# alpa-projects/alpa

Hardware: AMD Instinct MI355X
Metric: model_tflops_aggregate (higher is better)
Workload: dtype bf16; 1 GPU; model=GPT-2.6B, hidden=2560, layers=32, heads=32, vocab=51200, global_batch=32, seq_len=1024, num_micro_batches=1, parallelism=dp1, hip_graph=True

## Files before the change

### alpa_amd/ops/csrc/attention.hip

```cpp
#include "common.h"
#include "launchers.h"

#define ATTN_BLOCK_K 64
#define ATTN_FWD_THREADS 512
#define ATTN_BWD_THREADS 512

struct AttnStrides {
  int64_t qb, qh, qs;
  int64_t kb, kh, ks;
  int64_t vb, vh, vs;
  int64_t ob, oh, os;
};

static AttnStrides attn_strides(const int64_t* s) {
  return {s[0], s[1], s[2], s[3], s[4], s[5],
          s[6], s[7], s[8], s[9], s[10], s[11]};
}

__device__ inline int xcd_swizzle(int flat, int total) {
  constexpr int NXCD = 8;
  if (total % NXCD != 0) return flat;
  return (flat % NXCD) * (total / NXCD) + flat / NXCD;
}

template <int Dp, bool AL = false, bool VL = false>
__global__ __launch_bounds__(ATTN_FWD_THREADS) void attn_fwd_kernel(
    const short* __restrict__ q, const short* __restrict__ k,
    const short* __restrict__ v, short* __restrict__ o,
    float* __restrict__ lse_out, int H, int S, int Skv, int D, float scale,
    int causal, const float* __restrict__ alibi,
    const int* __restrict__ kv_lens, AttnStrides st) {
  constexpr bool DB = Dp <= 128;
  constexpr int NT = ATTN_FWD_THREADS;
  constexpr int KSTEPS_QK = Dp / 32;
  constexpr int NTILES = ATTN_BLOCK_K / 16;
  constexpr int DTILES = Dp / 16;
  constexpr int LP = 4;
  constexpr int NW = NT / 64;
  constexpr int GPR = Dp / 8;
  constexpr int TOTAL_G = ATTN_BLOCK_K * GPR;
  constexpr int G_PER_T = (TOTAL_G + NT - 1) / NT;

  const int flat_ = xcd_swizzle(
      (int)(blockIdx.y * gridDim.x + blockIdx.x),
      (int)(gridDim.x * gridDim.y));
  const int qb_raw = flat_ % (int)gridDim.x;
  const int qb = causal ? ((int)gridDim.x - 1 - qb_raw) : qb_raw;
  const int bh = flat_ / (int)gridDim.x;
  const int batch = bh / H, head = bh % H;
  const int wave = threadIdx.x >> 6;
  const int lane = threadIdx.x & 63;
  const int lo = lane & 15;
  const int hi = lane >> 4;

  const short* qp = q + batch * st.qb + head * st.qh;
  const short* kp = k + batch * st.kb + head * st.kh;
  const short* vp = v + batch * st.vb + head * st.vh;
  short* op = o + batch * st.ob + head * st.oh;
  const int q_row0 = qb * (16 * NW) + wave * 16;

  __shared__ short k_lds[DB ? 2 : 1][ATTN_BLOCK_K][Dp + LP];
  __shared__ short vt_lds[DB ? 2 : 1][Dp][ATTN_BLOCK_K + LP];
  __shared__ short p_lds[NW][16][ATTN_BLOCK_K + LP];

  bf16x8 q_frag[KSTEPS_QK];
  {
    int row = min(q_row0 + lo, S - 1);
#pragma unroll
    for (int ks = 0; ks < KSTEPS_QK; ++ks) {
      int col = ks * 32 + hi * 8;
      bf16x8 z = {0, 0, 0, 0, 0, 0, 0, 0};
      q_frag[ks] = z;
      if (col + 8 <= D)
        q_frag[ks] =
            *reinterpret_cast<const bf16x8*>(qp + (int64_t)row * st.qs + col);
    }
  }

  float m_state = -INFINITY, l_state = 0.f;
  f32x4 o_acc[DTILES];
#pragma unroll
  for (int dt = 0; dt < DTILES; ++dt) o_acc[dt] = f32x4{0.f, 0.f, 0.f, 0.f};

  const int kv_limit =
      causal ? min(Skv, qb * (16 * NW) + 16 * NW) : Skv;
  const int n_tiles = (kv_limit + ATTN_BLOCK_K - 1) / ATTN_BLOCK_K;
  const int my_q = q_row0 + lo;
  const int my_skv = VL ? kv_lens[batch] : Skv;
  const float al_slope = AL ? alibi[bh % H] : 0.f;
  const int al_qoff = my_skv - S;

  bf16x8 kreg[2 * G_PER_T], vreg[2 * G_PER_T];
  auto issue_loads = [&](int tile) {
#pragma unroll
    for (int it = 0; it < G_PER_T; ++it) {
      int t = threadIdx.x + it * NT;
      bf16x8 z = {0, 0, 0, 0, 0, 0, 0, 0};
      kreg[2 * it] = z; kreg[2 * it + 1] = z;
      vreg[2 * it] = z; vreg[2 * it + 1] = z;
      if (t < TOTAL_G / 2) {
        int kvr = (t / GPR) * 2, dg = (t % GPR) * 8;
#pragma unroll
        for (int u = 0; u < 2; ++u) {
          int src = tile * ATTN_BLOCK_K + kvr + u;
          if (src < Skv && dg + 8 <= D) {
            kreg[2 * it + u] = *reinterpret_cast<const bf16x8*>(
                kp + (int64_t)src * st.ks + dg);
            vreg[2 * it + u] = *reinterpret_cast<const bf16x8*>(
                vp + (int64_t)src * st.vs + dg);
          }
        }
      }
    }
  };
  auto write_tile = [&](int buf) {
#pragma unroll
    for (int it = 0; it < G_PER_T; ++it) {
      int t = threadIdx.x + it * NT;
      if (t < TOTAL_G / 2) {
        int kvr = (t / GPR) * 2, dg = (t % GPR) * 8;
        *reinterpret_cast<bf16x8*>(&k_lds[buf][kvr][dg]) = kreg[2 * it];
        *reinterpret_cast<bf16x8*>(&k_lds[buf][kvr + 1][dg]) =
            kreg[2 * it + 1];
#pragma unroll
        for (int j = 0; j < 8; ++j) {
          short2 pr;
          pr.x = vreg[2 * it][j];
          pr.y = vreg[2 * it + 1][j];
          *reinterpret_cast<short2*>(&vt_lds[buf][dg + j][kvr]) = pr;
        }
      }
    }
  };

  auto advance = [&](int ti, int cur) {
    if (ti + 1 >= n_tiles) return;
    if (DB) {
      write_tile(1 - cur);
      __syncthreads();
    } else {
      __syncthreads();
      issue_loads(ti + 1);
      write_tile(0);
      __syncthreads();
    }
  };

  if (n_tiles > 0) {
    issue_loads(0);
    write_tile(0);
    __syncthreads();
  }

  for (int ti = 0; ti < n_tiles; ++ti) {
    const int kvb = ti * ATTN_BLOCK_K;
    const int cur = DB ? (ti & 1) : 0;
    if (DB && ti + 1 < n_tiles) issue_loads(ti + 1);

    if (causal && kvb > q_row0 + 15) {
      advance(ti, cur);
      continue;
    }

__builtin_amdgcn_s_setprio(1);
    f32x4 s_acc[NTILES];
#pragma unroll
    for (int nt = 0; nt < NTILES; ++nt) {
      f32x4 acc = {0.f, 0.f, 0.f, 0.f};
#pragma unroll
      for (int ks = 0; ks < KSTEPS_QK; ++ks) {
        bf16x8 a = *reinterpret_cast<const bf16x8*>(
            &k_lds[cur][nt * 16 + lo][ks * 32 + hi * 8]);
        acc = __builtin_amdgcn_mfma_f32_16x16x32_bf16(a, q_frag[ks], acc, 0,
                                                      0, 0);
      }
      s_acc[nt] = acc;
    }
    __builtin_amdgcn_s_setprio(0);

    float tile_max = -INFINITY;
#pragma unroll
    for (int nt = 0; nt < NTILES; ++nt) {
#pragma unroll
      for (int r = 0; r < 4; ++r) {
        int kv_idx = kvb + nt * 16 + hi * 4 + r;
        float sv = s_acc[nt][r] * scale;
        if (AL)
          sv = fmaf(al_slope, (float)(kv_idx - my_q - al_qoff), sv);
        bool masked = (kv_idx >= my_skv) || (causal && kv_idx > my_q) ||
                      (my_q >= S);
        sv = masked ? -INFINITY : sv;
        s_acc[nt][r] = sv;
        tile_max = fmaxf(tile_max, sv);
      }
    }
    tile_max = fmaxf(tile_max, __shfl_xor(tile_max, 16, 64));
    tile_max = fmaxf(tile_max, __shfl_xor(tile_max, 32, 64));

    constexpr float DEFER_THR = 8.0f;
    if (!__all(tile_max <= m_state + DEFER_THR)) {
      float m_new = fmaxf(m_state, tile_max);
      float alpha = (m_state == -INFINITY) ? 0.f : __expf(m_state - m_new);
      m_state = m_new;
      l_state *= alpha;
#pragma unroll
      for (int dt = 0; dt < DTILES; ++dt) {
        o_acc[dt][0] *= alpha; o_acc[dt][1] *= alpha;
        o_acc[dt][2] *= alpha; o_acc[dt][3] *= alpha;
      }
    }
    float part = 0.f;
#pragma unroll
    for (int nt = 0; nt < NTILES; ++nt) {
      bf16x4 pk;
#pragma unroll
      for (int r = 0; r < 4; ++r) {
        float pval = (s_acc[nt][r] == -INFINITY)
                         ? 0.f
                         : __expf(s_acc[nt][r] - m_state);
        part += pval;
        pk[r] = f2bf(pval);
      }
      *reinterpret_cast<bf16x4*>(&p_lds[wave][lo][nt * 16 + hi * 4]) = pk;
    }
    part += __shfl_xor(part, 16, 64);
    part += __shfl_xor(part, 32, 64);
    l_state += part;

__builtin_amdgcn_s_setprio(1);
#pragma unroll
    for (int ks = 0; ks < ATTN_BLOCK_K / 32; ++ks) {
      bf16x8 b = *reinterpret_cast<const bf16x8*>(
          &p_lds[wave][lo][ks * 32 + hi * 8]);
#pragma unroll
      for (int dt = 0; dt < DTILES; ++dt) {
        bf16x8 a = *reinterpret_cast<const bf16x8*>(
            &vt_lds[cur][dt * 16 + lo][ks * 32 + hi * 8]);
        o_acc[dt] =
            __builtin_amdgcn_mfma_f32_16x16x32_bf16(a, b, o_acc[dt], 0, 0, 0);
      }
    }
    __builtin_amdgcn_s_setprio(0);

    advance(ti, cur);
  }

  {
    int q_idx = q_row0 + lo;
    if (q_idx < S) {
      float inv_l = (l_state > 0.f) ? 1.0f / l_state : 0.f;
#pragma unroll
      for (int dt = 0; dt < DTILES; ++dt) {
#pragma unroll
        for (int r = 0; r < 4; ++r) {
          int col = dt * 16 + hi * 4 + r;
          if (col < D)
            op[(int64_t)q_idx * st.os + col] = f2bf(o_acc[dt][r] * inv_l);
        }
      }
      if (hi == 0 && lse_out != nullptr)
        lse_out[(int64_t)bh * S + q_idx] =
            (l_state > 0.f) ? m_state + __logf(l_state) : -INFINITY;
    }
  }
}

extern "C" {

hipError_t launch_attn_fwd(const void* q, const void* k, const void* v,
                           void* o, float* lse, int64_t B, int64_t H,
                           int64_t S, int64_t Skv, int64_t D, float scale,
                           int causal, const float* alibi,
                           const int* kv_lens, const int64_t* strides,
                           hipStream_t stream) {
  const AttnStrides st = attn_strides(strides);
  dim3 grid((uint32_t)ceil_div(S, 16 * (ATTN_FWD_THREADS / 64)),
            (uint32_t)(B * H));
  dim3 block(ATTN_FWD_THREADS);
#define FWD_LAUNCH(DP, ALB, VLB)                                           \
  attn_fwd_kernel<DP, ALB, VLB><<<grid, block, 0, stream>>>(               \
      (const short*)q, (const short*)k, (const short*)v, (short*)o, lse,   \
      (int)H, (int)S, (int)Skv, (int)D, scale, causal, alibi, kv_lens, st)
#define FWD_DISPATCH(DP)                                                   \
  do {                                                                     \
    if (alibi && kv_lens) FWD_LAUNCH(DP, true, true);                      \
    else if (alibi) FWD_LAUNCH(DP, true, false);                           \
    else if (kv_lens) FWD_LAUNCH(DP, false, true);                         \
    else FWD_LAUNCH(DP, false, false);                                     \
  } while (0)
  if (D <= 64) {
    FWD_DISPATCH(64);
  } else if (D <= 96) {
    FWD_DISPATCH(96);
  } else if (D <= 128) {
    FWD_DISPATCH(128);
  } else if (D <= 256 && !alibi && !kv_lens) {
    FWD_LAUNCH(256, false, false);
  } else {
    return hipErrorInvalidValue;
  }
#undef FWD_DISPATCH
#undef FWD_LAUNCH
  return hipGetLastError();
}

}


struct AttnBwdStrides {
  int64_t qb, qh, qs;
  int64_t kb, kh, ks;
  int64_t vb, vh, vs;
  int64_t dob, doh, dos;
  int64_t dqb, dqh, dqs;
  int64_t dkb, dkh, dks;
  int64_t dvb, dvh, dvs;
};

static AttnBwdStrides attn_bwd_strides(const int64_t* s) {
  return {s[0],  s[1],  s[2],  s[3],  s[4],  s[5],  s[6],
          s[7],  s[8],  s[9],  s[10], s[11], s[12], s[13],
          s[14], s[15], s[16], s[17], s[18], s[19], s[20]};
}

__global__ void attn_bwd_preprocess_kernel(const short* __restrict__ dout,
                                           const short* __restrict__ o,
                                           float* __restrict__ delta,
                                           int64_t rows, int H, int S, int D,
                                           int64_t dob, int64_t doh,
                                           int64_t dos, int64_t ob,
                                           int64_t oh, int64_t os) {
  int64_t row = (int64_t)blockIdx.x * (blockDim.x >> 4) + (threadIdx.x >> 4);
  if (row >= rows) return;
  int lane16 = threadIdx.x & 15;
  int64_t sidx = row % S, h = (row / S) % H, b = row / ((int64_t)S * H);
  const short* dr = dout + b * dob + h * doh + sidx * dos;
  const short* orow = o + b * ob + h * oh + sidx * os;
  float s = 0.f;
  for (int i = lane16 * 8; i + 8 <= D; i += 16 * 8) {
    bf16x8 dv = *reinterpret_cast<const bf16x8*>(dr + i);
    bf16x8 ov = *reinterpret_cast<const bf16x8*>(orow + i);
#pragma unroll
    for (int j = 0; j < 8; ++j) s += bf2f(dv[j]) * bf2f(ov[j]);
  }
  if (lane16 == 0)
    for (int i = (D / 8) * 8; i < D; ++i)
      s += bf2f(dr[i]) * bf2f(orow[i]);
#pragma unroll
  for (int off = 8; off > 0; off >>= 1) s += __shfl_xor(s, off, 64);
  if (lane16 == 0) delta[row] = s;
}

template <int Dp, bool AL = false>
__global__ __launch_bounds__(ATTN_BWD_THREADS) void attn_bwd_dq_kernel(
    const short* __restrict__ q, const short* __restrict__ k,
    const short* __restrict__ v, const short* __restrict__ dout,
    const float* __restrict__ lse, const float* __restrict__ delta,
    short* __restrict__ dq, int H, int S, int Skv, int D, float scale,
    int causal, const float* __restrict__ alibi, AttnBwdStrides st) {
  constexpr int KD = Dp / 32;
  constexpr int NT = 4;
  constexpr int DT = Dp / 16;
  constexpr int LP = 4;
  constexpr int NW = ATTN_BWD_THREADS / 64;
  constexpr int GPR = Dp / 8;
  constexpr int PAIRS = 32 * GPR;

  const int flat_ = xcd_swizzle(
      (int)(blockIdx.y * gridDim.x + blockIdx.x),
      (int)(gridDim.x * gridDim.y));
  const int qb_raw = flat_ % (int)gridDim.x;
  const int qb = causal ? ((int)gridDim.x - 1 - qb_raw) : qb_raw;
  const int bh = flat_ / (int)gridDim.x;
  const int batch = bh / H, head = bh % H;
  const int wave = threadIdx.x >> 6;
  const int lane = threadIdx.x & 63;
  const int lo = lane & 15, hi = lane >> 4;

  const short* qp = q + batch * st.qb + head * st.qh;
  const short* kp = k + batch * st.kb + head * st.kh;
  const short* vp = v + batch * st.vb + head * st.vh;
  const short* dop = dout + batch * st.dob + head * st.doh;
  short* dqp = dq + batch * st.dqb + head * st.dqh;
  const int q_row0 = qb * (16 * NW) + wave * 16;

  __shared__ short k_lds[64][Dp + LP];
  __shared__ short kt_lds[Dp][64 + LP];
  __shared__ short v_lds[64][Dp + LP];
  __shared__ short p_lds[NW][16][64 + LP];

  bf16x8 q_frag[KD], do_frag[KD];
  {
    int row = min(q_row0 + lo, S - 1);
#pragma unroll
    for (int ks = 0; ks < KD; ++ks) {
      int col = ks * 32 + hi * 8;
      bf16x8 z = {0, 0, 0, 0, 0, 0, 0, 0};
      q_frag[ks] = z;
      do_frag[ks] = z;
      if (col + 8 <= D) {
        q_frag[ks] = *reinterpret_cast<const bf16x8*>(
            qp + (int64_t)row * st.qs + col);
        do_frag[ks] = *reinterpret_cast<const bf16x8*>(
            dop + (int64_t)row * st.dos + col);
      }
    }
  }
  float lse_r[4], delta_r[4];
#pragma unroll
  for (int r = 0; r < 4; ++r) {
    int qi = q_row0 + hi * 4 + r;
    lse_r[r] = (qi < S) ? lse[(int64_t)bh * S + qi] : 0.f;
    delta_r[r] = (qi < S) ? delta[(int64_t)bh * S + qi] : 0.f;
  }
  const float al_slope = AL ? alibi[bh % H] : 0.f;

  f32x4 dq_acc[DT];
#pragma unroll
  for (int dt = 0; dt < DT; ++dt) dq_acc[dt] = f32x4{0.f, 0.f, 0.f, 0.f};

  const int kv_limit = causal ? min(Skv, qb * (16 * NW) + 16 * NW) : Skv;
  const int n_tiles = (kv_limit + 63) / 64;

  bf16x8 kreg[2], vreg[2];
  auto issue_loads = [&](int tile) {
    int t = threadIdx.x;
    bf16x8 z = {0, 0, 0, 0, 0, 0, 0, 0};
    kreg[0] = kreg[1] = vreg[0] = vreg[1] = z;
    if (t < PAIRS) {
      int kvr = (t / GPR) * 2, dg = (t % GPR) * 8;
#pragma unroll
      for (int u = 0; u < 2; ++u) {
        int src = tile * 64 + kvr + u;
        if (src < Skv && dg + 8 <= D) {
          kreg[u] = *reinterpret_cast<const bf16x8*>(
              kp + (int64_t)src * st.ks + dg);
          vreg[u] = *reinterpret_cast<const bf16x8*>(
              vp + (int64_t)src * st.vs + dg);
        }
      }
    }
  };
  auto write_tile = [&]() {
    int t = threadIdx.x;
    if (t < PAIRS) {
      int kvr = (t / GPR) * 2, dg = (t % GPR) * 8;
      *reinterpret_cast<bf16x8*>(&k_lds[kvr][dg]) = kreg[0];
      *reinterpret_cast<bf16x8*>(&k_lds[kvr + 1][dg]) = kreg[1];
      *reinterpret_cast<bf16x8*>(&v_lds[kvr][dg]) = vreg[0];
      *reinterpret_cast<bf16x8*>(&v_lds[kvr + 1][dg]) = vreg[1];
#pragma unroll
      for (int j = 0; j < 8; ++j) {
        short2 pr;
        pr.x = kreg[0][j];
        pr.y = kreg[1][j];
        *reinterpret_cast<short2*>(&kt_lds[dg + j][kvr]) = pr;
      }
    }
  };

  if (n_tiles > 0) {
    issue_loads(0);
    write_tile();
    __syncthreads();
  }

  for (int ti = 0; ti < n_tiles; ++ti) {
    const int kvb = ti * 64;
    if (ti + 1 < n_tiles) issue_loads(ti + 1);

    if (causal && kvb > q_row0 + 15) {
      __syncthreads();
      if (ti + 1 < n_tiles) { write_tile(); __syncthreads(); }
      continue;
    }

__builtin_amdgcn_s_setprio(1);
    f32x4 s_acc[NT], dp_acc[NT];
#pragma unroll
    for (int nt = 0; nt < NT; ++nt) {
      f32x4 sa = {0.f, 0.f, 0.f, 0.f}, da = {0.f, 0.f, 0.f, 0.f};
#pragma unroll
      for (int ks = 0; ks < KD; ++ks) {
        bf16x8 bk = *reinterpret_cast<const bf16x8*>(
            &k_lds[nt * 16 + lo][ks * 32 + hi * 8]);
        bf16x8 bv = *reinterpret_cast<const bf16x8*>(
            &v_lds[nt * 16 + lo][ks * 32 + hi * 8]);
        sa = __builtin_amdgcn_mfma_f32_16x16x32_bf16(q_frag[ks], bk, sa, 0,
                                                     0, 0);
        da = __builtin_amdgcn_mfma_f32_16x16x32_bf16(do_frag[ks], bv, da, 0,
                                                     0, 0);
      }
      s_acc[nt] = sa;
      dp_acc[nt] = da;
    }
    __builtin_amdgcn_s_setprio(0);

#pragma unroll
    for (int nt = 0; nt < NT; ++nt) {
      int kv_idx = kvb + nt * 16 + lo;
#pragma unroll
      for (int r = 0; r < 4; ++r) {
        int q_idx = q_row0 + hi * 4 + r;
        bool masked = (kv_idx >= Skv) || (causal && kv_idx > q_idx) ||
                      (q_idx >= S);
        float sraw = s_acc[nt][r] * scale;
        if (AL) sraw = fmaf(al_slope, (float)(kv_idx - q_idx), sraw);
        float pv = masked ? 0.f : __expf(sraw - lse_r[r]);
        float ds = pv * (dp_acc[nt][r] - delta_r[r]) * scale;
        p_lds[wave][hi * 4 + r][nt * 16 + lo] = f2bf(ds);
      }
    }

__builtin_amdgcn_s_setprio(1);
#pragma unroll
    for (int ks = 0; ks < 2; ++ks) {
      bf16x8 a = *reinterpret_cast<const bf16x8*>(
          &p_lds[wave][lo][ks * 32 + hi * 8]);
#pragma unroll
      for (int dt = 0; dt < DT; ++dt) {
        bf16x8 b = *reinterpret_cast<const bf16x8*>(
            &kt_lds[dt * 16 + lo][ks * 32 + hi * 8]);
        dq_acc[dt] = __builtin_amdgcn_mfma_f32_16x16x32_bf16(
            a, b, dq_acc[dt], 0, 0, 0);
      }
    }
    __builtin_amdgcn_s_setprio(0);

    __syncthreads();
    if (ti + 1 < n_tiles) {
      write_tile();
      __syncthreads();
    }
  }

#pragma unroll
  for (int r = 0; r < 4; ++r) {
    int q_idx = q_row0 + hi * 4 + r;
    if (q_idx >= S) continue;
#pragma unroll
    for (int dt = 0; dt < DT; ++dt) {
      int col = dt * 16 + lo;
      if (col < D)
        dqp[(int64_t)q_idx * st.dqs + col] = f2bf(dq_acc[dt][r]);
    }
  }
}

template <int Dp, bool AL = false>
__global__ __launch_bounds__(ATTN_BWD_THREADS) void attn_bwd_dkv_kernel(
    const short* __restrict__ q, const short* __restrict__ k,
    const short* __restrict__ v, const short* __restrict__ dout,
    const float* __restrict__ lse, const float* __restrict__ delta,
    short* __restrict__ dk, short* __restrict__ dv, int H, int S, int Skv,
    int D, float scale, int causal, const float* __restrict__ alibi,
    AttnBwdStrides st) {
  constexpr int KD = Dp / 32;
  constexpr int NT = 4;
  constexpr int DT = Dp / 16;
  constexpr int LP = 4;
  constexpr int NW = ATTN_BWD_THREADS / 64;
  constexpr int GPR = Dp / 8;
  constexpr int PAIRS = 32 * GPR;

  const int flat_ = xcd_swizzle(
      (int)(blockIdx.y * gridDim.x + blockIdx.x),
      (int)(gridDim.x * gridDim.y));
  const int kvb_idx = flat_ % (int)gridDim.x;
  const int bh = flat_ / (int)gridDim.x;
  const int batch = bh / H, head = bh % H;
  const int wave = threadIdx.x >> 6;
  const int lane = threadIdx.x & 63;
  const int lo = lane & 15, hi = lane >> 4;

  const short* qp = q + batch * st.qb + head * st.qh;
  const short* kp = k + batch * st.kb + head * st.kh;
  const short* vp = v + batch * st.vb + head * st.vh;
  const short* dop = dout + batch * st.dob + head * st.doh;
  short* dkp = dk + batch * st.dkb + head * st.dkh;
  short* dvp = dv + batch * st.dvb + head * st.dvh;
  const int kv_row0 = kvb_idx * (16 * NW) + wave * 16;
  const float al_slope = AL ? alibi[bh % H] : 0.f;

  __shared__ short q_lds[64][Dp + LP];
  __shared__ short do_lds[64][Dp + LP];
  __shared__ short qt_lds[Dp][64 + LP];
  __shared__ short dot_lds[Dp][64 + LP];
  __shared__ short p_lds[NW][16][64 + LP];
  __shared__ float lse_lds[64];
  __shared__ float delta_lds[64];

  bf16x8 k_frag[KD], v_frag[KD];
  {
    int row = min(kv_row0 + lo, Skv - 1);
#pragma unroll
    for (int ks = 0; ks < KD; ++ks) {
      int col = ks * 32 + hi * 8;
      bf16x8 z = {0, 0, 0, 0, 0, 0, 0, 0};
      k_frag[ks] = z;
      v_frag[ks] = z;
      if (col + 8 <= D) {
        k_frag[ks] = *reinterpret_cast<const bf16x8*>(
            kp + (int64_t)row * st.ks + col);
        v_frag[ks] = *reinterpret_cast<const bf16x8*>(
            vp + (int64_t)row * st.vs + col);
      }
    }
  }

  f32x4 dk_acc[DT], dv_acc[DT];
#pragma unroll
  for (int dt = 0; dt < DT; ++dt) {
    dk_acc[dt] = f32x4{0.f, 0.f, 0.f, 0.f};
    dv_acc[dt] = f32x4{0.f, 0.f, 0.f, 0.f};
  }

  const int q_start = causal ? kvb_idx * (16 * NW) / 64 * 64 : 0;
  const int n_tiles = (S - q_start + 63) / 64;

  bf16x8 qreg[2], doreg[2];
  float lse_reg, delta_reg;
  auto issue_loads = [&](int tile) {
    int t = threadIdx.x;
    bf16x8 z = {0, 0, 0, 0, 0, 0, 0, 0};
    qreg[0] = qreg[1] = doreg[0] = doreg[1] = z;
    int qb0 = q_start + tile * 64;
    if (t < PAIRS) {
      int qr = (t / GPR) * 2, dg = (t % GPR) * 8;
#pragma unroll
      for (int u = 0; u < 2; ++u) {
        int src = qb0 + qr + u;
        if (src < S && dg + 8 <= D) {
          qreg[u] = *reinterpret_cast<const bf16x8*>(
              qp + (int64_t)src * st.qs + dg);
          doreg[u] = *reinterpret_cast<const bf16x8*>(
              dop + (int64_t)src * st.dos + dg);
        }
      }
    }
    lse_reg = delta_reg = 0.f;
    if (t < 64) {
      int src = qb0 + t;
      if (src < S) {
        lse_reg = lse[(int64_t)bh * S + src];
        delta_reg = delta[(int64_t)bh * S + src];
      }
    }
  };
  auto write_tile = [&]() {
    int t = threadIdx.x;
    if (t < PAIRS) {
      int qr = (t / GPR) * 2, dg = (t % GPR) * 8;
      *reinterpret_cast<bf16x8*>(&q_lds[qr][dg]) = qreg[0];
      *reinterpret_cast<bf16x8*>(&q_lds[qr + 1][dg]) = qreg[1];
      *reinterpret_cast<bf16x8*>(&do_lds[qr][dg]) = doreg[0];
      *reinterpret_cast<bf16x8*>(&do_lds[qr + 1][dg]) = doreg[1];
#pragma unroll
      for (int j = 0; j < 8; ++j) {
        short2 pq, pd;
        pq.x = qreg[0][j];
        pq.y = qreg[1][j];
        pd.x = doreg[0][j];
        pd.y = doreg[1][j];
        *reinterpret_cast<short2*>(&qt_lds[dg + j][qr]) = pq;
        *reinterpret_cast<short2*>(&dot_lds[dg + j][qr]) = pd;
      }
    }
    if (t < 64) {
      lse_lds[t] = lse_reg;
      delta_lds[t] = delta_reg;
    }
  };

  if (n_tiles > 0) {
    issue_loads(0);
    write_tile();
    __syncthreads();
  }

  for (int ti = 0; ti < n_tiles; ++ti) {
    const int qb0 = q_start + ti * 64;
    if (ti + 1 < n_tiles) issue_loads(ti + 1);

    if (causal && qb0 + 63 < kv_row0) {
      __syncthreads();
      if (ti + 1 < n_tiles) { write_tile(); __syncthreads(); }
      continue;
    }

__builtin_amdgcn_s_setprio(1);
    f32x4 st_acc[NT], dpt_acc[NT];
#pragma unroll
    for (int nt = 0; nt < NT; ++nt) {
      f32x4 sa = {0.f, 0.f, 0.f, 0.f}, da = {0.f, 0.f, 0.f, 0.f};
#pragma unroll
      for (int ks = 0; ks < KD; ++ks) {
        bf16x8 bq = *reinterpret_cast<const bf16x8*>(
            &q_lds[nt * 16 + lo][ks * 32 + hi * 8]);
        bf16x8 bd = *reinterpret_cast<const bf16x8*>(
            &do_lds[nt * 16 + lo][ks * 32 + hi * 8]);
        sa = __builtin_amdgcn_mfma_f32_16x16x32_bf16(k_frag[ks], bq, sa, 0,
                                                     0, 0);
        da = __builtin_amdgcn_mfma_f32_16x16x32_bf16(v_frag[ks], bd, da, 0,
                                                     0, 0);
      }
      st_acc[nt] = sa;
      dpt_acc[nt] = da;
    }
    __builtin_amdgcn_s_setprio(0);

    short dst_pk[NT][4];
#pragma unroll
    for (int nt = 0; nt < NT; ++nt) {
      int q_idx = qb0 + nt * 16 + lo;
#pragma unroll
      for (int r = 0; r < 4; ++r) {
        int kv_idx = kv_row0 + hi * 4 + r;
        bool masked = (q_idx >= S) || (kv_idx >= Skv) ||
                      (causal && kv_idx > q_idx);
        float sraw = st_acc[nt][r] * scale;
        if (AL) sraw = fmaf(al_slope, (float)(kv_idx - q_idx), sraw);
        float pv = masked ? 0.f : __expf(sraw - lse_lds[nt * 16 + lo]);
        p_lds[wave][hi * 4 + r][nt * 16 + lo] = f2bf(pv);
        dst_pk[nt][r] =
            f2bf(pv * (dpt_acc[nt][r] - delta_lds[nt * 16 + lo]) * scale);
      }
    }

__builtin_amdgcn_s_setprio(1);
#pragma unroll
    for (int ks = 0; ks < 2; ++ks) {
      bf16x8 a = *reinterpret_cast<const bf16x8*>(
          &p_lds[wave][lo][ks * 32 + hi * 8]);
#pragma unroll
      for (int dt = 0; dt < DT; ++dt) {
        bf16x8 b = *reinterpret_cast<const bf16x8*>(
            &dot_lds[dt * 16 + lo][ks * 32 + hi * 8]);
        dv_acc[dt] = __builtin_amdgcn_mfma_f32_16x16x32_bf16(
            a, b, dv_acc[dt], 0, 0, 0);
      }
#pragma unroll
      for (int nt = 2 * ks; nt < 2 * ks + 2; ++nt)
#pragma unroll
        for (int r = 0; r < 4; ++r)
          p_lds[wave][hi * 4 + r][nt * 16 + lo] = dst_pk[nt][r];
    }
    __builtin_amdgcn_s_setprio(0);

__builtin_amdgcn_s_setprio(1);
#pragma unroll
    for (int ks = 0; ks < 2; ++ks) {
      bf16x8 a = *reinterpret_cast<const bf16x8*>(
          &p_lds[wave][lo][ks * 32 + hi * 8]);
#pragma unroll
      for (int dt = 0; dt < DT; ++dt) {
        bf16x8 b = *reinterpret_cast<const bf16x8*>(
            &qt_lds[dt * 16 + lo][ks * 32 + hi * 8]);
        dk_acc[dt] = __builtin_amdgcn_mfma_f32_16x16x32_bf16(
            a, b, dk_acc[dt], 0, 0, 0);
      }
    }
    __builtin_amdgcn_s_setprio(0);

    __syncthreads();
    if (ti + 1 < n_tiles) {
      write_tile();
      __syncthreads();
    }
  }

#pragma unroll
  for (int r = 0; r < 4; ++r) {
    int kv_idx = kv_row0 + hi * 4 + r;
    if (kv_idx >= Skv) continue;
#pragma unroll
    for (int dt = 0; dt < DT; ++dt) {
      int col = dt * 16 + lo;
      if (col < D) {
        dkp[(int64_t)kv_idx * st.dks + col] = f2bf(dk_acc[dt][r]);
        dvp[(int64_t)kv_idx * st.dvs + col] = f2bf(dv_acc[dt][r]);
      }
    }
  }
}

extern "C" {

hipError_t launch_attn_bwd(const void* q, const void* k, const void* v,
                           const void* o, const void* dout,
                           const float* lse, float* delta_ws, void* dq,
                           void* dk, void* dv, int64_t B, int64_t H,
                           int64_t S, int64_t Skv, int64_t D, float scale,
                           int causal, const float* alibi,
                           const int64_t* strides, hipStream_t stream) {
  if (D > 128) return hipErrorInvalidValue;
  const AttnBwdStrides st = attn_bwd_strides(strides);
  int64_t rows = B * H * S;
  {
    dim3 block(256);
    dim3 grid((uint32_t)ceil_div(rows, 16));
    attn_bwd_preprocess_kernel<<<grid, block, 0, stream>>>(
        (const short*)dout, (const short*)o, delta_ws, rows, (int)H, (int)S,
        (int)D, st.dob, st.doh, st.dos, strides[21], strides[22],
        strides[23]);
  }
  static hipStream_t side_stream = nullptr;
  static hipEvent_t ev_fork = nullptr, ev_join = nullptr;
  if (side_stream == nullptr) {
    hipStreamCreateWithFlags(&side_stream, hipStreamNonBlocking);
    hipEventCreateWithFlags(&ev_fork, hipEventDisableTiming);
    hipEventCreateWithFlags(&ev_join, hipEventDisableTiming);
  }
  hipEventRecord(ev_fork, stream);
  hipStreamWaitEvent(side_stream, ev_fork, 0);
  dim3 block(ATTN_BWD_THREADS);
  dim3 grid_q((uint32_t)ceil_div(S, 16 * (ATTN_BWD_THREADS / 64)),
              (uint32_t)(B * H));
  dim3 grid_kv((uint32_t)ceil_div(Skv, 16 * (ATTN_BWD_THREADS / 64)),
               (uint32_t)(B * H));
#define LAUNCH_BWD_T(DP, ALB)                                              \
  do {                                                                     \
    attn_bwd_dq_kernel<DP, ALB><<<grid_q, block, 0, side_stream>>>(        \
        (const short*)q, (const short*)k, (const short*)v,                 \
        (const short*)dout, lse, delta_ws, (short*)dq, (int)H, (int)S,     \
        (int)Skv, (int)D, scale, causal, alibi, st);                       \
    attn_bwd_dkv_kernel<DP, ALB><<<grid_kv, block, 0, stream>>>(           \
        (const short*)q, (const short*)k, (const short*)v,                 \
        (const short*)dout, lse, delta_ws, (short*)dk, (short*)dv, (int)H, \
        (int)S, (int)Skv, (int)D, scale, causal, alibi, st);               \
  } while (0)
#define LAUNCH_BWD(DP)                                                     \
  do {                                                                     \
    if (alibi) LAUNCH_BWD_T(DP, true);                                     \
    else LAUNCH_BWD_T(DP, false);                                          \
  } while (0)
  if (D <= 64) {
    LAUNCH_BWD(64);
  } else if (D <= 96) {
    LAUNCH_BWD(96);
  } else {
    LAUNCH_BWD(128);
  }
#undef LAUNCH_BWD
#undef LAUNCH_BWD_T
  hipEventRecord(ev_join, side_stream);
  hipStreamWaitEvent(stream, ev_join, 0);
  return hipGetLastError();
}

}
```

### alpa_amd/ops/csrc/common.h

```cpp
#pragma once

#include <hip/hip_runtime.h>
#include <hip/hip_bf16.h>

#include <cstdint>

#define WAVE_SIZE 64

using bf16 = __hip_bfloat16;

typedef short bf16x8 __attribute__((ext_vector_type(8)));
typedef short bf16x4 __attribute__((ext_vector_type(4)));
typedef float f32x4 __attribute__((ext_vector_type(4)));
typedef float f32x16 __attribute__((ext_vector_type(16)));

__device__ __forceinline__ float bf2f(short raw) {
  union {
    float f;
    uint32_t u;
  } cvt;
  cvt.u = (uint32_t)(uint16_t)raw << 16;
  return cvt.f;
}

__device__ __forceinline__ short f2bf(float f) {
  union {
    float f;
    uint32_t u;
  } cvt;
  cvt.f = f;
  uint32_t lsb = (cvt.u >> 16) & 1;
  cvt.u += 0x7fff + lsb;
  return (short)(cvt.u >> 16);
}

__device__ __forceinline__ float wave_reduce_sum(float v) {
#pragma unroll
  for (int off = 32; off > 0; off >>= 1) v += __shfl_xor(v, off, 64);
  return v;
}

__device__ __forceinline__ float wave_reduce_max(float v) {
#pragma unroll
  for (int off = 32; off > 0; off >>= 1)
    v = fmaxf(v, __shfl_xor(v, off, 64));
  return v;
}

__device__ __forceinline__ float block_reduce_sum(float v, float* buf) {
  int lane = threadIdx.x & 63;
  int wave = threadIdx.x >> 6;
  int nwaves = blockDim.x >> 6;
  v = wave_reduce_sum(v);
  if (lane == 0) buf[wave] = v;
  __syncthreads();
  float r = (lane < nwaves) ? buf[lane] : 0.0f;
  r = wave_reduce_sum(r);
  __syncthreads();
  return r;
}

__device__ __forceinline__ float block_reduce_max(float v, float* buf) {
  int lane = threadIdx.x & 63;
  int wave = threadIdx.x >> 6;
  int nwaves = blockDim.x >> 6;
  v = wave_reduce_max(v);
  if (lane == 0) buf[wave] = v;
  __syncthreads();
  float r = (lane < nwaves) ? buf[lane] : -INFINITY;
  r = wave_reduce_max(r);
  __syncthreads();
  return r;
}

__host__ __forceinline__ int64_t ceil_div(int64_t a, int64_t b) {
  return (a + b - 1) / b;
}
```

Before: 836.8 TFLOPS.

## Rewrite attention backward kernels with multi-row waves and double-buffered LDS

```diff
diff --git a/alpa_amd/ops/csrc/attention.hip b/alpa_amd/ops/csrc/attention.hip
--- a/alpa_amd/ops/csrc/attention.hip
+++ b/alpa_amd/ops/csrc/attention.hip
@@ -3,7 +3,6 @@
 
 #define ATTN_BLOCK_K 64
 #define ATTN_FWD_THREADS 512
-#define ATTN_BWD_THREADS 512
 
 struct AttnStrides {
   int64_t qb, qh, qs;
@@ -15,12 +14,6 @@
 static AttnStrides attn_strides(const int64_t* s) {
   return {s[0], s[1], s[2], s[3], s[4], s[5],
           s[6], s[7], s[8], s[9], s[10], s[11]};
-}
-
-__device__ inline int xcd_swizzle(int flat, int total) {
-  constexpr int NXCD = 8;
-  if (total % NXCD != 0) return flat;
-  return (flat % NXCD) * (total / NXCD) + flat / NXCD;
 }
 
 template <int Dp, bool AL = false, bool VL = false>
@@ -305,547 +298,3 @@
 }
 
 }
-
-
-struct AttnBwdStrides {
-  int64_t qb, qh, qs;
-  int64_t kb, kh, ks;
-  int64_t vb, vh, vs;
-  int64_t dob, doh, dos;
-  int64_t dqb, dqh, dqs;
-  int64_t dkb, dkh, dks;
-  int64_t dvb, dvh, dvs;
-};
-
-static AttnBwdStrides attn_bwd_strides(const int64_t* s) {
-  return {s[0],  s[1],  s[2],  s[3],  s[4],  s[5],  s[6],
-          s[7],  s[8],  s[9],  s[10], s[11], s[12], s[13],
-          s[14], s[15], s[16], s[17], s[18], s[19], s[20]};
-}
-
-__global__ void attn_bwd_preprocess_kernel(const short* __restrict__ dout,
-                                           const short* __restrict__ o,
-                                           float* __restrict__ delta,
-                                           int64_t rows, int H, int S, int D,
-                                           int64_t dob, int64_t doh,
-                                           int64_t dos, int64_t ob,
-                                           int64_t oh, int64_t os) {
-  int64_t row = (int64_t)blockIdx.x * (blockDim.x >> 4) + (threadIdx.x >> 4);
-  if (row >= rows) return;
-  int lane16 = threadIdx.x & 15;
-  int64_t sidx = row % S, h = (row / S) % H, b = row / ((int64_t)S * H);
-  const short* dr = dout + b * dob + h * doh + sidx * dos;
-  const short* orow = o + b * ob + h * oh + sidx * os;
-  float s = 0.f;
-  for (int i = lane16 * 8; i + 8 <= D; i += 16 * 8) {
-    bf16x8 dv = *reinterpret_cast<const bf16x8*>(dr + i);
-    bf16x8 ov = *reinterpret_cast<const bf16x8*>(orow + i);
-#pragma unroll
-    for (int j = 0; j < 8; ++j) s += bf2f(dv[j]) * bf2f(ov[j]);
-  }
-  if (lane16 == 0)
-    for (int i = (D / 8) * 8; i < D; ++i)
-      s += bf2f(dr[i]) * bf2f(orow[i]);
-#pragma unroll
-  for (int off = 8; off > 0; off >>= 1) s += __shfl_xor(s, off, 64);
-  if (lane16 == 0) delta[row] = s;
-}
-
-template <int Dp, bool AL = false>
-__global__ __launch_bounds__(ATTN_BWD_THREADS) void attn_bwd_dq_kernel(
-    const short* __restrict__ q, const short* __restrict__ k,
-    const short* __restrict__ v, const short* __restrict__ dout,
-    const float* __restrict__ lse, const float* __restrict__ delta,
-    short* __restrict__ dq, int H, int S, int Skv, int D, float scale,
-    int causal, const float* __restrict__ alibi, AttnBwdStrides st) {
-  constexpr int KD = Dp / 32;
-  constexpr int NT = 4;
-  constexpr int DT = Dp / 16;
-  constexpr int LP = 4;
-  constexpr int NW = ATTN_BWD_THREADS / 64;
-  constexpr int GPR = Dp / 8;
-  constexpr int PAIRS = 32 * GPR;
-
-  const int flat_ = xcd_swizzle(
-      (int)(blockIdx.y * gridDim.x + blockIdx.x),
-      (int)(gridDim.x * gridDim.y));
-  const int qb_raw = flat_ % (int)gridDim.x;
-  const int qb = causal ? ((int)gridDim.x - 1 - qb_raw) : qb_raw;
-  const int bh = flat_ / (int)gridDim.x;
-  const int batch = bh / H, head = bh % H;
-  const int wave = threadIdx.x >> 6;
-  const int lane = threadIdx.x & 63;
-  const int lo = lane & 15, hi = lane >> 4;
-
-  const short* qp = q + batch * st.qb + head * st.qh;
-  const short* kp = k + batch * st.kb + head * st.kh;
-  const short* vp = v + batch * st.vb + head * st.vh;
-  const short* dop = dout + batch * st.dob + head * st.doh;
-  short* dqp = dq + batch * st.dqb + head * st.dqh;
-  const int q_row0 = qb * (16 * NW) + wave * 16;
-
-  __shared__ short k_lds[64][Dp + LP];
-  __shared__ short kt_lds[Dp][64 + LP];
-  __shared__ short v_lds[64][Dp + LP];
-  __shared__ short p_lds[NW][16][64 + LP];
-
-  bf16x8 q_frag[KD], do_frag[KD];
-  {
-    int row = min(q_row0 + lo, S - 1);
-#pragma unroll
-    for (int ks = 0; ks < KD; ++ks) {
-      int col = ks * 32 + hi * 8;
-      bf16x8 z = {0, 0, 0, 0, 0, 0, 0, 0};
-      q_frag[ks] = z;
-      do_frag[ks] = z;
-      if (col + 8 <= D) {
-        q_frag[ks] = *reinterpret_cast<const bf16x8*>(
-            qp + (int64_t)row * st.qs + col);
-        do_frag[ks] = *reinterpret_cast<const bf16x8*>(
-            dop + (int64_t)row * st.dos + col);
-      }
-    }
-  }
-  float lse_r[4], delta_r[4];
-#pragma unroll
-  for (int r = 0; r < 4; ++r) {
-    int qi = q_row0 + hi * 4 + r;
-    lse_r[r] = (qi < S) ? lse[(int64_t)bh * S + qi] : 0.f;
-    delta_r[r] = (qi < S) ? delta[(int64_t)bh * S + qi] : 0.f;
-  }
-  const float al_slope = AL ? alibi[bh % H] : 0.f;
-
-  f32x4 dq_acc[DT];
-#pragma unroll
-  for (int dt = 0; dt < DT; ++dt) dq_acc[dt] = f32x4{0.f, 0.f, 0.f, 0.f};
-
-  const int kv_limit = causal ? min(Skv, qb * (16 * NW) + 16 * NW) : Skv;
-  const int n_tiles = (kv_limit + 63) / 64;
-
-  bf16x8 kreg[2], vreg[2];
-  auto issue_loads = [&](int tile) {
-    int t = threadIdx.x;
-    bf16x8 z = {0, 0, 0, 0, 0, 0, 0, 0};
-    kreg[0] = kreg[1] = vreg[0] = vreg[1] = z;
-    if (t < PAIRS) {
-      int kvr = (t / GPR) * 2, dg = (t % GPR) * 8;
-#pragma unroll
-      for (int u = 0; u < 2; ++u) {
-        int src = tile * 64 + kvr + u;
-        if (src < Skv && dg + 8 <= D) {
-          kreg[u] = *reinterpret_cast<const bf16x8*>(
-              kp + (int64_t)src * st.ks + dg);
-          vreg[u] = *reinterpret_cast<const bf16x8*>(
-              vp + (int64_t)src * st.vs + dg);
-        }
-      }
-    }
-  };
-  auto write_tile = [&]() {
-    int t = threadIdx.x;
-    if (t < PAIRS) {
-      int kvr = (t / GPR) * 2, dg = (t % GPR) * 8;
-      *reinterpret_cast<bf16x8*>(&k_lds[kvr][dg]) = kreg[0];
-      *reinterpret_cast<bf16x8*>(&k_lds[kvr + 1][dg]) = kreg[1];
-      *reinterpret_cast<bf16x8*>(&v_lds[kvr][dg]) = vreg[0];
-      *reinterpret_cast<bf16x8*>(&v_lds[kvr + 1][dg]) = vreg[1];
-#pragma unroll
-      for (int j = 0; j < 8; ++j) {
-        short2 pr;
-        pr.x = kreg[0][j];
-        pr.y = kreg[1][j];
-        *reinterpret_cast<short2*>(&kt_lds[dg + j][kvr]) = pr;
-      }
-    }
-  };
-
-  if (n_tiles > 0) {
-    issue_loads(0);
-    write_tile();
-    __syncthreads();
-  }
-
-  for (int ti = 0; ti < n_tiles; ++ti) {
-    const int kvb = ti * 64;
-    if (ti + 1 < n_tiles) issue_loads(ti + 1);
-
-    if (causal && kvb > q_row0 + 15) {
-      __syncthreads();
-      if (ti + 1 < n_tiles) { write_tile(); __syncthreads(); }
-      continue;
-    }
-
-__builtin_amdgcn_s_setprio(1);
-    f32x4 s_acc[NT], dp_acc[NT];
-#pragma unroll
-    for (int nt = 0; nt < NT; ++nt) {
-      f32x4 sa = {0.f, 0.f, 0.f, 0.f}, da = {0.f, 0.f, 0.f, 0.f};
-#pragma unroll
-      for (int ks = 0; ks < KD; ++ks) {
-        bf16x8 bk = *reinterpret_cast<const bf16x8*>(
-            &k_lds[nt * 16 + lo][ks * 32 + hi * 8]);
-        bf16x8 bv = *reinterpret_cast<const bf16x8*>(
-            &v_lds[nt * 16 + lo][ks * 32 + hi * 8]);
-        sa = __builtin_amdgcn_mfma_f32_16x16x32_bf16(q_frag[ks], bk, sa, 0,
-                                                     0, 0);
-        da = __builtin_amdgcn_mfma_f32_16x16x32_bf16(do_frag[ks], bv, da, 0,
-                                                     0, 0);
-      }
-      s_acc[nt] = sa;
-      dp_acc[nt] = da;
-    }
-    __builtin_amdgcn_s_setprio(0);
-
-#pragma unroll
-    for (int nt = 0; nt < NT; ++nt) {
-      int kv_idx = kvb + nt * 16 + lo;
-#pragma unroll
-      for (int r = 0; r < 4; ++r) {
-        int q_idx = q_row0 + hi * 4 + r;
-        bool masked = (kv_idx >= Skv) || (causal && kv_idx > q_idx) ||
-                      (q_idx >= S);
-        float sraw = s_acc[nt][r] * scale;
-        if (AL) sraw = fmaf(al_slope, (float)(kv_idx - q_idx), sraw);
-        float pv = masked ? 0.f : __expf(sraw - lse_r[r]);
-        float ds = pv * (dp_acc[nt][r] - delta_r[r]) * scale;
-        p_lds[wave][hi * 4 + r][nt * 16 + lo] = f2bf(ds);
-      }
-    }
-
-__builtin_amdgcn_s_setprio(1);
-#pragma unroll
-    for (int ks = 0; ks < 2; ++ks) {
-      bf16x8 a = *reinterpret_cast<const bf16x8*>(
-          &p_lds[wave][lo][ks * 32 + hi * 8]);
-#pragma unroll
-      for (int dt = 0; dt < DT; ++dt) {
-        bf16x8 b = *reinterpret_cast<const bf16x8*>(
-            &kt_lds[dt * 16 + lo][ks * 32 + hi * 8]);
-        dq_acc[dt] = __builtin_amdgcn_mfma_f32_16x16x32_bf16(
-            a, b, dq_acc[dt], 0, 0, 0);
-      }
-    }
-    __builtin_amdgcn_s_setprio(0);
-
-    __syncthreads();
-    if (ti + 1 < n_tiles) {
-      write_tile();
-      __syncthreads();
-    }
-  }
-
-#pragma unroll
-  for (int r = 0; r < 4; ++r) {
-    int q_idx = q_row0 + hi * 4 + r;
-    if (q_idx >= S) continue;
-#pragma unroll
-    for (int dt = 0; dt < DT; ++dt) {
-      int col = dt * 16 + lo;
-      if (col < D)
-        dqp[(int64_t)q_idx * st.dqs + col] = f2bf(dq_acc[dt][r]);
-    }
-  }
-}
-
-template <int Dp, bool AL = false>
-__global__ __launch_bounds__(ATTN_BWD_THREADS) void attn_bwd_dkv_kernel(
-    const short* __restrict__ q, const short* __restrict__ k,
-    const short* __restrict__ v, const short* __restrict__ dout,
-    const float* __restrict__ lse, const float* __restrict__ delta,
-    short* __restrict__ dk, short* __restrict__ dv, int H, int S, int Skv,
-    int D, float scale, int causal, const float* __restrict__ alibi,
-    AttnBwdStrides st) {
-  constexpr int KD = Dp / 32;
-  constexpr int NT = 4;
-  constexpr int DT = Dp / 16;
-  constexpr int LP = 4;
-  constexpr int NW = ATTN_BWD_THREADS / 64;
-  constexpr int GPR = Dp / 8;
-  constexpr int PAIRS = 32 * GPR;
-
-  const int flat_ = xcd_swizzle(
-      (int)(blockIdx.y * gridDim.x + blockIdx.x),
-      (int)(gridDim.x * gridDim.y));
-  const int kvb_idx = flat_ % (int)gridDim.x;
-  const int bh = flat_ / (int)gridDim.x;
-  const int batch = bh / H, head = bh % H;
-  const int wave = threadIdx.x >> 6;
-  const int lane = threadIdx.x & 63;
-  const int lo = lane & 15, hi = lane >> 4;
-
-  const short* qp = q + batch * st.qb + head * st.qh;
-  const short* kp = k + batch * st.kb + head * st.kh;
-  const short* vp = v + batch * st.vb + head * st.vh;
-  const short* dop = dout + batch * st.dob + head * st.doh;
-  short* dkp = dk + batch * st.dkb + head * st.dkh;
-  short* dvp = dv + batch * st.dvb + head * st.dvh;
-  const int kv_row0 = kvb_idx * (16 * NW) + wave * 16;
-  const float al_slope = AL ? alibi[bh % H] : 0.f;
-
-  __shared__ short q_lds[64][Dp + LP];
-  __shared__ short do_lds[64][Dp + LP];
-  __shared__ short qt_lds[Dp][64 + LP];
-  __shared__ short dot_lds[Dp][64 + LP];
-  __shared__ short p_lds[NW][16][64 + LP];
-  __shared__ float lse_lds[64];
-  __shared__ float delta_lds[64];
-
-  bf16x8 k_frag[KD], v_frag[KD];
-  {
-    int row = min(kv_row0 + lo, Skv - 1);
-#pragma unroll
-    for (int ks = 0; ks < KD; ++ks) {
-      int col = ks * 32 + hi * 8;
-      bf16x8 z = {0, 0, 0, 0, 0, 0, 0, 0};
-      k_frag[ks] = z;
-      v_frag[ks] = z;
-      if (col + 8 <= D) {
-        k_frag[ks] = *reinterpret_cast<const bf16x8*>(
-            kp + (int64_t)row * st.ks + col);
-        v_frag[ks] = *reinterpret_cast<const bf16x8*>(
-            vp + (int64_t)row * st.vs + col);
-      }
-    }
-  }
-
-  f32x4 dk_acc[DT], dv_acc[DT];
-#pragma unroll
-  for (int dt = 0; dt < DT; ++dt) {
-    dk_acc[dt] = f32x4{0.f, 0.f, 0.f, 0.f};
-    dv_acc[dt] = f32x4{0.f, 0.f, 0.f, 0.f};
-  }
-
-  const int q_start = causal ? kvb_idx * (16 * NW) / 64 * 64 : 0;
-  const int n_tiles = (S - q_start + 63) / 64;
-
-  bf16x8 qreg[2], doreg[2];
-  float lse_reg, delta_reg;
-  auto issue_loads = [&](int tile) {
-    int t = threadIdx.x;
-    bf16x8 z = {0, 0, 0, 0, 0, 0, 0, 0};
-    qreg[0] = qreg[1] = doreg[0] = doreg[1] = z;
-    int qb0 = q_start + tile * 64;
-    if (t < PAIRS) {
-      int qr = (t / GPR) * 2, dg = (t % GPR) * 8;
-#pragma unroll
-      for (int u = 0; u < 2; ++u) {
-        int src = qb0 + qr + u;
-        if (src < S && dg + 8 <= D) {
-          qreg[u] = *reinterpret_cast<const bf16x8*>(
-              qp + (int64_t)src * st.qs + dg);
-          doreg[u] = *reinterpret_cast<const bf16x8*>(
-              dop + (int64_t)src * st.dos + dg);
-        }
-      }
-    }
-    lse_reg = delta_reg = 0.f;
-    if (t < 64) {
-      int src = qb0 + t;
-      if (src < S) {
-        lse_reg = lse[(int64_t)bh * S + src];
-        delta_reg = delta[(int64_t)bh * S + src];
-      }
-    }
-  };
-  auto write_tile = [&]() {
-    int t = threadIdx.x;
-    if (t < PAIRS) {
-      int qr = (t / GPR) * 2, dg = (t % GPR) * 8;
-      *reinterpret_cast<bf16x8*>(&q_lds[qr][dg]) = qreg[0];
-      *reinterpret_cast<bf16x8*>(&q_lds[qr + 1][dg]) = qreg[1];
-      *reinterpret_cast<bf16x8*>(&do_lds[qr][dg]) = doreg[0];
-      *reinterpret_cast<bf16x8*>(&do_lds[qr + 1][dg]) = doreg[1];
-#pragma unroll
-      for (int j = 0; j < 8; ++j) {
-        short2 pq, pd;
-        pq.x = qreg[0][j];
-        pq.y = qreg[1][j];
-        pd.x = doreg[0][j];
-        pd.y = doreg[1][j];
-        *reinterpret_cast<short2*>(&qt_lds[dg + j][qr]) = pq;
-        *reinterpret_cast<short2*>(&dot_lds[dg + j][qr]) = pd;
-      }
-    }
-    if (t < 64) {
-      lse_lds[t] = lse_reg;
-      delta_lds[t] = delta_reg;
-    }
-  };
-
-  if (n_tiles > 0) {
-    issue_loads(0);
-    write_tile();
-    __syncthreads();
-  }
-
-  for (int ti = 0; ti < n_tiles; ++ti) {
-    const int qb0 = q_start + ti * 64;
-    if (ti + 1 < n_tiles) issue_loads(ti + 1);
-
-    if (causal && qb0 + 63 < kv_row0) {
-      __syncthreads();
-      if (ti + 1 < n_tiles) { write_tile(); __syncthreads(); }
-      continue;
-    }
-
-__builtin_amdgcn_s_setprio(1);
-    f32x4 st_acc[NT], dpt_acc[NT];
-#pragma unroll
-    for (int nt = 0; nt < NT; ++nt) {
-      f32x4 sa = {0.f, 0.f, 0.f, 0.f}, da = {0.f, 0.f, 0.f, 0.f};
-#pragma unroll
-      for (int ks = 0; ks < KD; ++ks) {
-        bf16x8 bq = *reinterpret_cast<const bf16x8*>(
-            &q_lds[nt * 16 + lo][ks * 32 + hi * 8]);
-        bf16x8 bd = *reinterpret_cast<const bf16x8*>(
-            &do_lds[nt * 16 + lo][ks * 32 + hi * 8]);
-        sa = __builtin_amdgcn_mfma_f32_16x16x32_bf16(k_frag[ks], bq, sa, 0,
-                                                     0, 0);
-        da = __builtin_amdgcn_mfma_f32_16x16x32_bf16(v_frag[ks], bd, da, 0,
-                                                     0, 0);
-      }
-      st_acc[nt] = sa;
-      dpt_acc[nt] = da;
-    }
-    __builtin_amdgcn_s_setprio(0);
-
-    short dst_pk[NT][4];
-#pragma unroll
-    for (int nt = 0; nt < NT; ++nt) {
-      int q_idx = qb0 + nt * 16 + lo;
-#pragma unroll
-      for (int r = 0; r < 4; ++r) {
-        int kv_idx = kv_row0 + hi * 4 + r;
-        bool masked = (q_idx >= S) || (kv_idx >= Skv) ||
-                      (causal && kv_idx > q_idx);
-        float sraw = st_acc[nt][r] * scale;
-        if (AL) sraw = fmaf(al_slope, (float)(kv_idx - q_idx), sraw);
-        float pv = masked ? 0.f : __expf(sraw - lse_lds[nt * 16 + lo]);
-        p_lds[wave][hi * 4 + r][nt * 16 + lo] = f2bf(pv);
-        dst_pk[nt][r] =
-            f2bf(pv * (dpt_acc[nt][r] - delta_lds[nt * 16 + lo]) * scale);
-      }
-    }
-
-__builtin_amdgcn_s_setprio(1);
-#pragma unroll
-    for (int ks = 0; ks < 2; ++ks) {
-      bf16x8 a = *reinterpret_cast<const bf16x8*>(
-          &p_lds[wave][lo][ks * 32 + hi * 8]);
-#pragma unroll
-      for (int dt = 0; dt < DT; ++dt) {
-        bf16x8 b = *reinterpret_cast<const bf16x8*>(
-            &dot_lds[dt * 16 + lo][ks * 32 + hi * 8]);
-        dv_acc[dt] = __builtin_amdgcn_mfma_f32_16x16x32_bf16(
-            a, b, dv_acc[dt], 0, 0, 0);
-      }
-#pragma unroll
-      for (int nt = 2 * ks; nt < 2 * ks + 2; ++nt)
-#pragma unroll
-        for (int r = 0; r < 4; ++r)
-          p_lds[wave][hi * 4 + r][nt * 16 + lo] = dst_pk[nt][r];
-    }
-    __builtin_amdgcn_s_setprio(0);
-
-__builtin_amdgcn_s_setprio(1);
-#pragma unroll
-    for (int ks = 0; ks < 2; ++ks) {
-      bf16x8 a = *reinterpret_cast<const bf16x8*>(
-          &p_lds[wave][lo][ks * 32 + hi * 8]);
-#pragma unroll
-      for (int dt = 0; dt < DT; ++dt) {
-        bf16x8 b = *reinterpret_cast<const bf16x8*>(
-            &qt_lds[dt * 16 + lo][ks * 32 + hi * 8]);
-        dk_acc[dt] = __builtin_amdgcn_mfma_f32_16x16x32_bf16(
-            a, b, dk_acc[dt], 0, 0, 0);
-      }
-    }
-    __builtin_amdgcn_s_setprio(0);
-
-    __syncthreads();
-    if (ti + 1 < n_tiles) {
-      write_tile();
-      __syncthreads();
-    }
-  }
-
-#pragma unroll
-  for (int r = 0; r < 4; ++r) {
-    int kv_idx = kv_row0 + hi * 4 + r;
-    if (kv_idx >= Skv) continue;
-#pragma unroll
-    for (int dt = 0; dt < DT; ++dt) {
-      int col = dt * 16 + lo;
-      if (col < D) {
-        dkp[(int64_t)kv_idx * st.dks + col] = f2bf(dk_acc[dt][r]);
-        dvp[(int64_t)kv_idx * st.dvs + col] = f2bf(dv_acc[dt][r]);
-      }
-    }
-  }
-}
-
-extern "C" {
-
-hipError_t launch_attn_bwd(const void* q, const void* k, const void* v,
-                           const void* o, const void* dout,
-                           const float* lse, float* delta_ws, void* dq,
-                           void* dk, void* dv, int64_t B, int64_t H,
-                           int64_t S, int64_t Skv, int64_t D, float scale,
-                           int causal, const float* alibi,
-                           const int64_t* strides, hipStream_t stream) {
-  if (D > 128) return hipErrorInvalidValue;
-  const AttnBwdStrides st = attn_bwd_strides(strides);
-  int64_t rows = B * H * S;
-  {
-    dim3 block(256);
-    dim3 grid((uint32_t)ceil_div(rows, 16));
-    attn_bwd_preprocess_kernel<<<grid, block, 0, stream>>>(
-        (const short*)dout, (const short*)o, delta_ws, rows, (int)H, (int)S,
-        (int)D, st.dob, st.doh, st.dos, strides[21], strides[22],
-        strides[23]);
-  }
-  static hipStream_t side_stream = nullptr;
-  static hipEvent_t ev_fork = nullptr, ev_join = nullptr;
-  if (side_stream == nullptr) {
-    hipStreamCreateWithFlags(&side_stream, hipStreamNonBlocking);
-    hipEventCreateWithFlags(&ev_fork, hipEventDisableTiming);
-    hipEventCreateWithFlags(&ev_join, hipEventDisableTiming);
-  }
-  hipEventRecord(ev_fork, stream);
-  hipStreamWaitEvent(side_stream, ev_fork, 0);
-  dim3 block(ATTN_BWD_THREADS);
-  dim3 grid_q((uint32_t)ceil_div(S, 16 * (ATTN_BWD_THREADS / 64)),
-              (uint32_t)(B * H));
-  dim3 grid_kv((uint32_t)ceil_div(Skv, 16 * (ATTN_BWD_THREADS / 64)),
-               (uint32_t)(B * H));
-#define LAUNCH_BWD_T(DP, ALB)                                              \
-  do {                                                                     \
-    attn_bwd_dq_kernel<DP, ALB><<<grid_q, block, 0, side_stream>>>(        \
-        (const short*)q, (const short*)k, (const short*)v,                 \
-        (const short*)dout, lse, delta_ws, (short*)dq, (int)H, (int)S,     \
-        (int)Skv, (int)D, scale, causal, alibi, st);                       \
-    attn_bwd_dkv_kernel<DP, ALB><<<grid_kv, block, 0, stream>>>(           \
-        (const short*)q, (const short*)k, (const short*)v,                 \
-        (const short*)dout, lse, delta_ws, (short*)dk, (short*)dv, (int)H, \
-        (int)S, (int)Skv, (int)D, scale, causal, alibi, st);               \
-  } while (0)
-#define LAUNCH_BWD(DP)                                                     \
-  do {                                                                     \
-    if (alibi) LAUNCH_BWD_T(DP, true);                                     \
-    else LAUNCH_BWD_T(DP, false);                                          \
-  } while (0)
-  if (D <= 64) {
-    LAUNCH_BWD(64);
-  } else if (D <= 96) {
-    LAUNCH_BWD(96);
-  } else {
-    LAUNCH_BWD(128);
-  }
-#undef LAUNCH_BWD
-#undef LAUNCH_BWD_T
-  hipEventRecord(ev_join, side_stream);
-  hipStreamWaitEvent(stream, ev_join, 0);
-  return hipGetLastError();
-}
-
-}
diff --git a/alpa_amd/ops/csrc/attention_bwd.hip b/alpa_amd/ops/csrc/attention_bwd.hip
--- /dev/null
+++ b/alpa_amd/ops/csrc/attention_bwd.hip
@@ -0,0 +1,577 @@
+#include <climits>
+
+#include "common.h"
+#include "launchers.h"
+
+struct AttnBwdStrides {
+  int64_t qb, qh, qs;
+  int64_t kb, kh, ks;
+  int64_t vb, vh, vs;
+  int64_t dob, doh, dos;
+  int64_t dqb, dqh, dqs;
+  int64_t dkb, dkh, dks;
+  int64_t dvb, dvh, dvs;
+};
+
+static AttnBwdStrides attn_bwd_strides(const int64_t* s) {
+  return {s[0],  s[1],  s[2],  s[3],  s[4],  s[5],  s[6],
+          s[7],  s[8],  s[9],  s[10], s[11], s[12], s[13],
+          s[14], s[15], s[16], s[17], s[18], s[19], s[20]};
+}
+
+__global__ void attn_bwd_preprocess_kernel(const short* __restrict__ dout,
+                                           const short* __restrict__ o,
+                                           float* __restrict__ delta,
+                                           int64_t rows, int H, int S, int D,
+                                           int64_t dob, int64_t doh,
+                                           int64_t dos, int64_t ob,
+                                           int64_t oh, int64_t os) {
+  int64_t row = (int64_t)blockIdx.x * (blockDim.x >> 4) + (threadIdx.x >> 4);
+  if (row >= rows) return;
+  int lane16 = threadIdx.x & 15;
+  int64_t sidx = row % S, h = (row / S) % H, b = row / ((int64_t)S * H);
+  const short* dr = dout + b * dob + h * doh + sidx * dos;
+  const short* orow = o + b * ob + h * oh + sidx * os;
+  float s = 0.f;
+  for (int i = lane16 * 8; i + 8 <= D; i += 16 * 8) {
+    bf16x8 dv = *reinterpret_cast<const bf16x8*>(dr + i);
+    bf16x8 ov = *reinterpret_cast<const bf16x8*>(orow + i);
+#pragma unroll
+    for (int j = 0; j < 8; ++j) s += bf2f(dv[j]) * bf2f(ov[j]);
+  }
+  if (lane16 == 0)
+    for (int i = (D / 8) * 8; i < D; ++i)
+      s += bf2f(dr[i]) * bf2f(orow[i]);
+#pragma unroll
+  for (int off = 8; off > 0; off >>= 1) s += __shfl_xor(s, off, 64);
+  if (lane16 == 0) delta[row] = s;
+}
+
+template <int DK>
+struct BwdTile {
+  static_assert(DK % 16 == 0 && DK <= 128, "unsupported head-dim tile");
+  static constexpr int K32 = DK / 32;
+  static constexpr bool K16 = (DK % 32) != 0;
+  static constexpr int DT = DK / 16;
+  static constexpr int RS = K16 ? DK : DK + 16;
+  static constexpr int GPR = DK / 8;
+  static constexpr int GROUPS = 64 * GPR;
+  static_assert((RS / 2) % 16 == 8, "row must be an odd multiple of 8 dwords");
+};
+
+constexpr float ATTN_LOG2E = 1.4426950408889634f;
+
+typedef uint32_t u32x4 __attribute__((ext_vector_type(4)));
+typedef float f32x2 __attribute__((ext_vector_type(2)));
+typedef __bf16 bf16v2 __attribute__((ext_vector_type(2)));
+
+__device__ __forceinline__ uint32_t pack_bf16(float lo, float hi) {
+  f32x2 v = {lo, hi};
+  return __builtin_bit_cast(uint32_t, __builtin_convertvector(v, bf16v2));
+}
+
+template <int DK>
+struct RowFrag {
+  bf16x8 w[BwdTile<DK>::K32];
+  bf16x8 t;
+};
+
+template <int DK>
+__device__ __forceinline__ void load_row_frag(RowFrag<DK>& f,
+                                              const short* __restrict__ rowp,
+                                              int hi, int D) {
+  using T = BwdTile<DK>;
+#pragma unroll
+  for (int ks = 0; ks < T::K32; ++ks) {
+    int col = ks * 32 + hi * 8;
+    bf16x8 z = {0, 0, 0, 0, 0, 0, 0, 0};
+    f.w[ks] = z;
+    if (col + 8 <= D) f.w[ks] = *reinterpret_cast<const bf16x8*>(rowp + col);
+  }
+  bf16x8 z8 = {0, 0, 0, 0, 0, 0, 0, 0};
+  f.t = z8;
+  if (T::K16) {
+    int col = T::K32 * 32 + hi * 8;
+    if (hi < 2 && col + 8 <= D)
+      f.t = *reinterpret_cast<const bf16x8*>(rowp + col);
+  }
+}
+
+template <int DK, int RW>
+__device__ __forceinline__ void rows_x_frags(const short* row, int hi,
+                                             const RowFrag<DK> (&b)[RW],
+                                             f32x4 (&acc)[RW]) {
+  using T = BwdTile<DK>;
+  if (T::K16) {
+    bf16x8 a = *reinterpret_cast<const bf16x8*>(row + T::K32 * 32 +
+                                                (hi & 1) * 8);
+#pragma unroll
+    for (int rw = 0; rw < RW; ++rw)
+      acc[rw] = __builtin_amdgcn_mfma_f32_16x16x32_bf16(a, b[rw].t, acc[rw],
+                                                        0, 0, 0);
+  }
+#pragma unroll
+  for (int ks = 0; ks < T::K32; ++ks) {
+    bf16x8 a = *reinterpret_cast<const bf16x8*>(row + ks * 32 + hi * 8);
+#pragma unroll
+    for (int rw = 0; rw < RW; ++rw)
+      acc[rw] = __builtin_amdgcn_mfma_f32_16x16x32_bf16(a, b[rw].w[ks],
+                                                        acc[rw], 0, 0, 0);
+  }
+}
+
+typedef short __attribute__((address_space(3))) lds_short;
+typedef bf16x4 __attribute__((address_space(3))) lds_bf16x4;
+__device__ __forceinline__ bf16x4 lds_read_tr(const short* p) {
+  return __builtin_amdgcn_ds_read_tr16_b64_v4i16(
+      (lds_bf16x4*)(lds_short*)const_cast<short*>(p));
+}
+
+template <int DK, int RW>
+__device__ __forceinline__ void frags_x_cols(
+    const u32x4 (&a)[RW], const short* img, int lo, int hi,
+    f32x4 (&acc)[RW][BwdTile<DK>::DT]) {
+  using T = BwdTile<DK>;
+  const short* p = img + (4 * hi + (lo >> 2)) * T::RS + 4 * (lo & 3);
+#pragma unroll
+  for (int dt = 0; dt < T::DT; ++dt) {
+    bf16x4 b0 = lds_read_tr(p + dt * 16);
+    bf16x4 b1 = lds_read_tr(p + 16 * T::RS + dt * 16);
+    bf16x8 b = __builtin_shufflevector(b0, b1, 0, 1, 2, 3, 4, 5, 6, 7);
+#pragma unroll
+    for (int rw = 0; rw < RW; ++rw)
+      acc[rw][dt] = __builtin_amdgcn_mfma_f32_16x16x32_bf16(
+          __builtin_bit_cast(bf16x8, a[rw]), b, acc[rw][dt], 0, 0, 0);
+  }
+}
+
+template <int DK, int RW, int NW, bool AL = false>
+__global__ __launch_bounds__(NW * 64, 2) void attn_bwd_dq_kernel(
+    const short* __restrict__ q, const short* __restrict__ k,
+    const short* __restrict__ v, const short* __restrict__ dout,
+    const float* __restrict__ lse, const float* __restrict__ delta,
+    short* __restrict__ dq, int H, int S, int Skv, int D, float scale,
+    int causal, const float* __restrict__ alibi, AttnBwdStrides st) {
+  using T = BwdTile<DK>;
+  constexpr int NT = 4;
+  constexpr int NTHR = NW * 64;
+  constexpr int WROWS = 16 * RW;
+  constexpr int ROWS = NW * WROWS;
+  constexpr int G_IT = (T::GROUPS + NTHR - 1) / NTHR;
+
+  const int flat_ = xcd_swizzle(
+      (int)(blockIdx.y * gridDim.x + blockIdx.x),
+      (int)(gridDim.x * gridDim.y));
+  const int qb_raw = flat_ % (int)gridDim.x;
+  const int qb = causal ? ((int)gridDim.x - 1 - qb_raw) : qb_raw;
+  const int bh = flat_ / (int)gridDim.x;
+  const int batch = bh / H, head = bh % H;
+  const int wave = __builtin_amdgcn_readfirstlane(threadIdx.x >> 6);
+  const int lane = threadIdx.x & 63;
+  const int lo = lane & 15, hi = lane >> 4;
+
+  const short* qp = q + batch * st.qb + head * st.qh;
+  const short* kp = k + batch * st.kb + head * st.kh;
+  const short* vp = v + batch * st.vb + head * st.vh;
+  const short* dop = dout + batch * st.dob + head * st.doh;
+  short* dqp = dq + batch * st.dqb + head * st.dqh;
+  const int q_row0 = qb * ROWS + wave * WROWS;
+
+  __shared__ __attribute__((aligned(16))) short k_lds[2][64][T::RS];
+  __shared__ __attribute__((aligned(16))) short v_lds[2][64][T::RS];
+
+  RowFrag<DK> q_frag[RW], do_frag[RW];
+  float lse2_q[RW], delta_q[RW];
+#pragma unroll
+  for (int rw = 0; rw < RW; ++rw) {
+    int my_q = q_row0 + 16 * rw + lo;
+    int row = min(my_q, S - 1);
+    load_row_frag<DK>(q_frag[rw], qp + (int64_t)row * st.qs, hi, D);
+    load_row_frag<DK>(do_frag[rw], dop + (int64_t)row * st.dos, hi, D);
+    lse2_q[rw] =
+        (my_q < S) ? lse[(int64_t)bh * S + my_q] * ATTN_LOG2E : 0.f;
+    delta_q[rw] = (my_q < S) ? delta[(int64_t)bh * S + my_q] : 0.f;
+  }
+  const float scale2 = scale * ATTN_LOG2E;
+  const float al_slope2 = AL ? alibi[bh % H] * ATTN_LOG2E : 0.f;
+
+  int kv_end[RW];
+#pragma unroll
+  for (int rw = 0; rw < RW; ++rw) {
+    int my_q = q_row0 + 16 * rw + lo;
+    kv_end[rw] = (my_q >= S) ? 0 : (causal ? min(my_q + 1, Skv) : Skv);
+  }
+
+  f32x4 dq_acc[RW][T::DT];
+#pragma unroll
+  for (int rw = 0; rw < RW; ++rw)
+#pragma unroll
+    for (int dt = 0; dt < T::DT; ++dt)
+      dq_acc[rw][dt] = f32x4{0.f, 0.f, 0.f, 0.f};
+
+  const int kv_limit = causal ? min(Skv, qb * ROWS + ROWS) : Skv;
+  const int n_tiles = (kv_limit + 63) / 64;
+
+  bf16x8 kreg[G_IT], vreg[G_IT];
+  auto issue_loads = [&](int tile) {
+#pragma unroll
+    for (int it = 0; it < G_IT; ++it) {
+      int g = threadIdx.x + it * NTHR;
+      int row = g / T::GPR, dg = (g % T::GPR) * 8;
+      int src = tile * 64 + row;
+      bf16x8 z = {0, 0, 0, 0, 0, 0, 0, 0};
+      kreg[it] = z;
+      vreg[it] = z;
+      if (g < T::GROUPS && src < Skv && dg + 8 <= D) {
+        kreg[it] = *reinterpret_cast<const bf16x8*>(
+            kp + (int64_t)src * st.ks + dg);
+        vreg[it] = *reinterpret_cast<const bf16x8*>(
+            vp + (int64_t)src * st.vs + dg);
+      }
+    }
+  };
+  auto write_tile = [&](int buf) {
+#pragma unroll
+    for (int it = 0; it < G_IT; ++it) {
+      int g = threadIdx.x + it * NTHR;
+      int row = g / T::GPR, dg = (g % T::GPR) * 8;
+      if (g < T::GROUPS) {
+        *reinterpret_cast<bf16x8*>(&k_lds[buf][row][dg]) = kreg[it];
+        *reinterpret_cast<bf16x8*>(&v_lds[buf][row][dg]) = vreg[it];
+      }
+    }
+  };
+
+  if (n_tiles > 0) {
+    issue_loads(0);
+    write_tile(0);
+    __syncthreads();
+  }
+
+  for (int ti = 0; ti < n_tiles; ++ti) {
+    const int kvb = ti * 64;
+    const int cur = ti & 1;
+    const bool more = ti + 1 < n_tiles;
+    if (more) issue_loads(ti + 1);
+
+    if (!(causal && kvb > q_row0 + WROWS - 1)) {
+      __builtin_amdgcn_s_setprio(1);
+      u32x4 ds_a[RW][2];
+#pragma unroll
+      for (int nt = 0; nt < NT; ++nt) {
+        f32x4 sa[RW], da[RW];
+#pragma unroll
+        for (int rw = 0; rw < RW; ++rw) {
+          sa[rw] = f32x4{0.f, 0.f, 0.f, 0.f};
+          da[rw] = f32x4{0.f, 0.f, 0.f, 0.f};
+        }
+        rows_x_frags<DK, RW>(&k_lds[cur][nt * 16 + lo][0], hi, q_frag, sa);
+        rows_x_frags<DK, RW>(&v_lds[cur][nt * 16 + lo][0], hi, do_frag, da);
+#pragma unroll
+        for (int rw = 0; rw < RW; ++rw) {
+          const int my_q = q_row0 + 16 * rw + lo;
+          float ds[4];
+#pragma unroll
+          for (int r = 0; r < 4; ++r) {
+            int kv_idx = kvb + nt * 16 + hi * 4 + r;
+            float x = fmaf(sa[rw][r], scale2, -lse2_q[rw]);
+            if (AL) x = fmaf(al_slope2, (float)(kv_idx - my_q), x);
+            float pv = __builtin_amdgcn_exp2f(x);
+            pv = (kv_idx < kv_end[rw]) ? pv : 0.f;
+            ds[r] = pv * (da[rw][r] - delta_q[rw]) * scale;
+          }
+          ds_a[rw][nt >> 1][2 * (nt & 1)] = pack_bf16(ds[0], ds[1]);
+          ds_a[rw][nt >> 1][2 * (nt & 1) + 1] = pack_bf16(ds[2], ds[3]);
+        }
+      }
+#pragma unroll
+      for (int s = 0; s < 2; ++s) {
+        u32x4 a[RW];
+#pragma unroll
+        for (int rw = 0; rw < RW; ++rw) a[rw] = ds_a[rw][s];
+        frags_x_cols<DK, RW>(a, &k_lds[cur][32 * s][0], lo, hi, dq_acc);
+      }
+      __builtin_amdgcn_s_setprio(0);
+    }
+
+    if (more) write_tile(1 - cur);
+    __syncthreads();
+  }
+
+#pragma unroll
+  for (int rw = 0; rw < RW; ++rw) {
+#pragma unroll
+    for (int r = 0; r < 4; ++r) {
+      int q_idx = q_row0 + 16 * rw + hi * 4 + r;
+      if (q_idx >= S) continue;
+#pragma unroll
+      for (int dt = 0; dt < T::DT; ++dt) {
+        int col = dt * 16 + lo;
+        if (col < D)
+          dqp[(int64_t)q_idx * st.dqs + col] = f2bf(dq_acc[rw][dt][r]);
+      }
+    }
+  }
+}
+
+template <int DK, int RW, int NW, bool AL = false>
+__global__ __launch_bounds__(NW * 64, 2) void attn_bwd_dkv_kernel(
+    const short* __restrict__ q, const short* __restrict__ k,
+    const short* __restrict__ v, const short* __restrict__ dout,
+    const float* __restrict__ lse, const float* __restrict__ delta,
+    short* __restrict__ dk, short* __restrict__ dv, int H, int S, int Skv,
+    int D, float scale, int causal, const float* __restrict__ alibi,
+    AttnBwdStrides st) {
+  using T = BwdTile<DK>;
+  constexpr int NT = 4;
+  constexpr int NTHR = NW * 64;
+  constexpr int WROWS = 16 * RW;
+  constexpr int ROWS = NW * WROWS;
+  constexpr int G_IT = (T::GROUPS + NTHR - 1) / NTHR;
+  static_assert(NTHR >= 64, "threads 0..63 stage lse/delta");
+
+  const int flat_ = xcd_swizzle(
+      (int)(blockIdx.y * gridDim.x + blockIdx.x),
+      (int)(gridDim.x * gridDim.y));
+  const int kvb_idx = flat_ % (int)gridDim.x;
+  const int bh = flat_ / (int)gridDim.x;
+  const int batch = bh / H, head = bh % H;
+  const int wave = __builtin_amdgcn_readfirstlane(threadIdx.x >> 6);
+  const int lane = threadIdx.x & 63;
+  const int lo = lane & 15, hi = lane >> 4;
+
+  const short* qp = q + batch * st.qb + head * st.qh;
+  const short* kp = k + batch * st.kb + head * st.kh;
+  const short* vp = v + batch * st.vb + head * st.vh;
+  const short* dop = dout + batch * st.dob + head * st.doh;
+  short* dkp = dk + batch * st.dkb + head * st.dkh;
+  short* dvp = dv + batch * st.dvb + head * st.dvh;
+  const int kv_row0 = kvb_idx * ROWS + wave * WROWS;
+  const float scale2 = scale * ATTN_LOG2E;
+  const float al_slope2 = AL ? alibi[bh % H] * ATTN_LOG2E : 0.f;
+
+  __shared__ __attribute__((aligned(16))) short q_lds[2][64][T::RS];
+  __shared__ __attribute__((aligned(16))) short do_lds[2][64][T::RS];
+  __shared__ __attribute__((aligned(16))) float lse2_lds[2][64];
+  __shared__ __attribute__((aligned(16))) float delta_lds[2][64];
+
+  RowFrag<DK> k_frag[RW], v_frag[RW];
+#pragma unroll
+  for (int rw = 0; rw < RW; ++rw) {
+    int row = min(kv_row0 + 16 * rw + lo, Skv - 1);
+    load_row_frag<DK>(k_frag[rw], kp + (int64_t)row * st.ks, hi, D);
+    load_row_frag<DK>(v_frag[rw], vp + (int64_t)row * st.vs, hi, D);
+  }
+
+  int q_lo[RW];
+#pragma unroll
+  for (int rw = 0; rw < RW; ++rw) {
+    int my_kv = kv_row0 + 16 * rw + lo;
+    q_lo[rw] = (my_kv >= Skv) ? INT_MAX : (causal ? my_kv : 0);
+  }
+
+  f32x4 dk_acc[RW][T::DT], dv_acc[RW][T::DT];
+#pragma unroll
+  for (int rw = 0; rw < RW; ++rw)
+#pragma unroll
+    for (int dt = 0; dt < T::DT; ++dt) {
+      dk_acc[rw][dt] = f32x4{0.f, 0.f, 0.f, 0.f};
+      dv_acc[rw][dt] = f32x4{0.f, 0.f, 0.f, 0.f};
+    }
+
+  const int q_start = causal ? kvb_idx * ROWS / 64 * 64 : 0;
+  const int n_tiles = (S - q_start + 63) / 64;
+
+  bf16x8 qreg[G_IT], doreg[G_IT];
+  float lse_reg, delta_reg;
+  auto issue_loads = [&](int tile) {
+    int qb0 = q_start + tile * 64;
+#pragma unroll
+    for (int it = 0; it < G_IT; ++it) {
+      int g = threadIdx.x + it * NTHR;
+      int row = g / T::GPR, dg = (g % T::GPR) * 8;
+      int src = qb0 + row;
+      bf16x8 z = {0, 0, 0, 0, 0, 0, 0, 0};
+      qreg[it] = z;
+      doreg[it] = z;
+      if (g < T::GROUPS && src < S && dg + 8 <= D) {
+        qreg[it] = *reinterpret_cast<const bf16x8*>(
+            qp + (int64_t)src * st.qs + dg);
+        doreg[it] = *reinterpret_cast<const bf16x8*>(
+            dop + (int64_t)src * st.dos + dg);
+      }
+    }
+    lse_reg = delta_reg = 0.f;
+    if (threadIdx.x < 64) {
+      int src = qb0 + threadIdx.x;
+      if (src < S) {
+        lse_reg = lse[(int64_t)bh * S + src];
+        delta_reg = delta[(int64_t)bh * S + src];
+      }
+    }
+  };
+  auto write_tile = [&](int buf) {
+#pragma unroll
+    for (int it = 0; it < G_IT; ++it) {
+      int g = threadIdx.x + it * NTHR;
+      int row = g / T::GPR, dg = (g % T::GPR) * 8;
+      if (g < T::GROUPS) {
+        *reinterpret_cast<bf16x8*>(&q_lds[buf][row][dg]) = qreg[it];
+        *reinterpret_cast<bf16x8*>(&do_lds[buf][row][dg]) = doreg[it];
+      }
+    }
+    if (threadIdx.x < 64) {
+      lse2_lds[buf][threadIdx.x] = lse_reg * ATTN_LOG2E;
+      delta_lds[buf][threadIdx.x] = delta_reg;
+    }
+  };
+
+  if (n_tiles > 0) {
+    issue_loads(0);
+    write_tile(0);
+    __syncthreads();
+  }
+
+  for (int ti = 0; ti < n_tiles; ++ti) {
+    const int qb0 = q_start + ti * 64;
+    const int cur = ti & 1;
+    const bool more = ti + 1 < n_tiles;
+    if (more) issue_loads(ti + 1);
+
+    if (!(causal && qb0 + 63 < kv_row0)) {
+      __builtin_amdgcn_s_setprio(1);
+#pragma unroll
+      for (int s = 0; s < 2; ++s) {
+        u32x4 p_a[RW], ds_a[RW];
+#pragma unroll
+        for (int h = 0; h < 2; ++h) {
+          const int nt = 2 * s + h;
+          f32x4 sa[RW], da[RW];
+#pragma unroll
+          for (int rw = 0; rw < RW; ++rw) {
+            sa[rw] = f32x4{0.f, 0.f, 0.f, 0.f};
+            da[rw] = f32x4{0.f, 0.f, 0.f, 0.f};
+          }
+          rows_x_frags<DK, RW>(&q_lds[cur][nt * 16 + lo][0], hi, k_frag, sa);
+          rows_x_frags<DK, RW>(&do_lds[cur][nt * 16 + lo][0], hi, v_frag,
+                               da);
+          const f32x4 l4 = *reinterpret_cast<const f32x4*>(
+              &lse2_lds[cur][nt * 16 + hi * 4]);
+          const f32x4 d4 = *reinterpret_cast<const f32x4*>(
+              &delta_lds[cur][nt * 16 + hi * 4]);
+#pragma unroll
+          for (int rw = 0; rw < RW; ++rw) {
+            const int my_kv = kv_row0 + 16 * rw + lo;
+            float pv[4], ds[4];
+#pragma unroll
+            for (int r = 0; r < 4; ++r) {
+              int q_idx = qb0 + nt * 16 + hi * 4 + r;
+              float x = fmaf(sa[rw][r], scale2, -l4[r]);
+              if (AL) x = fmaf(al_slope2, (float)(my_kv - q_idx), x);
+              pv[r] = __builtin_amdgcn_exp2f(x);
+              pv[r] = (q_idx >= q_lo[rw]) ? pv[r] : 0.f;
+              ds[r] = pv[r] * (da[rw][r] - d4[r]) * scale;
+            }
+            p_a[rw][2 * h] = pack_bf16(pv[0], pv[1]);
+            p_a[rw][2 * h + 1] = pack_bf16(pv[2], pv[3]);
+            ds_a[rw][2 * h] = pack_bf16(ds[0], ds[1]);
+            ds_a[rw][2 * h + 1] = pack_bf16(ds[2], ds[3]);
+          }
+        }
+        frags_x_cols<DK, RW>(p_a, &do_lds[cur][32 * s][0], lo, hi, dv_acc);
+        frags_x_cols<DK, RW>(ds_a, &q_lds[cur][32 * s][0], lo, hi, dk_acc);
+      }
+      __builtin_amdgcn_s_setprio(0);
+    }
+
+    if (more) write_tile(1 - cur);
+    __syncthreads();
+  }
+
+#pragma unroll
+  for (int rw = 0; rw < RW; ++rw) {
+#pragma unroll
+    for (int r = 0; r < 4; ++r) {
+      int kv_idx = kv_row0 + 16 * rw + hi * 4 + r;
+      if (kv_idx >= Skv) continue;
+#pragma unroll
+      for (int dt = 0; dt < T::DT; ++dt) {
+        int col = dt * 16 + lo;
+        if (col < D) {
+          dkp[(int64_t)kv_idx * st.dks + col] = f2bf(dk_acc[rw][dt][r]);
+          dvp[(int64_t)kv_idx * st.dvs + col] = f2bf(dv_acc[rw][dt][r]);
+        }
+      }
+    }
+  }
+}
+
+extern "C" {
+
+hipError_t launch_attn_bwd(const void* q, const void* k, const void* v,
+                           const void* o, const void* dout,
+                           const float* lse, float* delta_ws, void* dq,
+                           void* dk, void* dv, int64_t B, int64_t H,
+                           int64_t S, int64_t Skv, int64_t D, float scale,
+                           int causal, const float* alibi,
+                           const int64_t* strides, hipStream_t stream) {
+  if (D > 128) return hipErrorInvalidValue;
+  const AttnBwdStrides st = attn_bwd_strides(strides);
+  int64_t rows = B * H * S;
+  {
+    dim3 block(256);
+    dim3 grid((uint32_t)ceil_div(rows, 16));
+    attn_bwd_preprocess_kernel<<<grid, block, 0, stream>>>(
+        (const short*)dout, (const short*)o, delta_ws, rows, (int)H, (int)S,
+        (int)D, st.dob, st.doh, st.dos, strides[21], strides[22],
+        strides[23]);
+  }
+  static hipStream_t side_stream = nullptr;
+  static hipEvent_t ev_fork = nullptr, ev_join = nullptr;
+  if (side_stream == nullptr) {
+    (void)hipStreamCreateWithFlags(&side_stream, hipStreamNonBlocking);
+    (void)hipEventCreateWithFlags(&ev_fork, hipEventDisableTiming);
+    (void)hipEventCreateWithFlags(&ev_join, hipEventDisableTiming);
+  }
+  (void)hipEventRecord(ev_fork, stream);
+  (void)hipStreamWaitEvent(side_stream, ev_fork, 0);
+  constexpr int BLOCK_ROWS = 128;
+  dim3 grid_q((uint32_t)ceil_div(S, BLOCK_ROWS), (uint32_t)(B * H));
+  dim3 grid_kv((uint32_t)ceil_div(Skv, BLOCK_ROWS), (uint32_t)(B * H));
+#define LAUNCH_BWD_T(DK, RWQ, NWQ, RWK, NWK, ALB)                          \
+  do {                                                                     \
+    static_assert(NWQ * RWQ * 16 == BLOCK_ROWS, "grid assumes 128 rows");  \
+    static_assert(NWK * RWK * 16 == BLOCK_ROWS, "grid assumes 128 rows");  \
+    attn_bwd_dq_kernel<DK, RWQ, NWQ, ALB>                                  \
+        <<<grid_q, dim3(NWQ * 64), 0, side_stream>>>(                      \
+            (const short*)q, (const short*)k, (const short*)v,             \
+            (const short*)dout, lse, delta_ws, (short*)dq, (int)H, (int)S, \
+            (int)Skv, (int)D, scale, causal, alibi, st);                   \
+    attn_bwd_dkv_kernel<DK, RWK, NWK, ALB>                                 \
+        <<<grid_kv, dim3(NWK * 64), 0, stream>>>(                          \
+            (const short*)q, (const short*)k, (const short*)v,             \
+            (const short*)dout, lse, delta_ws, (short*)dk, (short*)dv,     \
+            (int)H, (int)S, (int)Skv, (int)D, scale, causal, alibi, st);   \
+  } while (0)
+#define LAUNCH_BWD(DK, RWQ, NWQ, RWK, NWK)                                 \
+  do {                                                                     \
+    if (alibi) LAUNCH_BWD_T(DK, RWQ, NWQ, RWK, NWK, true);                 \
+    else LAUNCH_BWD_T(DK, RWQ, NWQ, RWK, NWK, false);                      \
+  } while (0)
+  if (D <= 64) {
+    LAUNCH_BWD(64, 2, 4, 2, 4);
+  } else if (D == 80) {
+    LAUNCH_BWD(80, 2, 4, 2, 4);
+  } else if (D <= 96) {
+    LAUNCH_BWD(96, 2, 4, 1, 8);
+  } else {
+    LAUNCH_BWD(128, 1, 8, 1, 8);
+  }
+#undef LAUNCH_BWD
+#undef LAUNCH_BWD_T
+  (void)hipEventRecord(ev_join, side_stream);
+  (void)hipStreamWaitEvent(stream, ev_join, 0);
+  return hipGetLastError();
+}
+
+}
diff --git a/alpa_amd/ops/csrc/common.h b/alpa_amd/ops/csrc/common.h
--- a/alpa_amd/ops/csrc/common.h
+++ b/alpa_amd/ops/csrc/common.h
@@ -73,6 +73,12 @@
   return r;
 }
 
+__device__ inline int xcd_swizzle(int flat, int total) {
+  constexpr int NXCD = 8;
+  if (total % NXCD != 0) return flat;
+  return (flat % NXCD) * (total / NXCD) + flat / NXCD;
+}
+
 __host__ __forceinline__ int64_t ceil_div(int64_t a, int64_t b) {
   return (a + b - 1) / b;
 }
```

Result: faster. 925.4 TFLOPS (median of 6 runs) (+10.6%).
